# semihkacmaz/CoNFiLD

Hardware: AMD Instinct MI355X
Metric: generated fields/sec (256-step sample + CNF decode), Case4 latent, 1/2/4/8 GPU (higher is better)
Workload: dtype f32

## Files before the change

confild_amd/csrc/diffusion.hip:

```cpp
#include <cmath>
#include <string>

#include "common.hpp"
#include "sampler.hpp"

namespace cfd {

struct Philox {
    static __device__ __forceinline__ uint4 round(uint4 c, uint2 k) {
        const uint64_t p0 = (uint64_t)0xD2511F53u * c.x;
        const uint64_t p1 = (uint64_t)0xCD9E8D57u * c.z;
        return make_uint4((uint32_t)(p1 >> 32) ^ c.y ^ k.x, (uint32_t)p1, (uint32_t)(p0 >> 32) ^ c.w ^ k.y,
                          (uint32_t)p0);
    }
    static __device__ __forceinline__ uint4 gen(uint64_t seed, uint64_t ctr_lo, uint64_t ctr_hi) {
        uint4 c = make_uint4((uint32_t)ctr_lo, (uint32_t)(ctr_lo >> 32), (uint32_t)ctr_hi, (uint32_t)(ctr_hi >> 32));
        uint2 k = make_uint2((uint32_t)seed, (uint32_t)(seed >> 32));
#pragma unroll
        for (int r = 0; r < 10; ++r) {
            c = round(c, k);
            k.x += 0x9E3779B9u;
            k.y += 0xBB67AE85u;
        }
        return c;
// ... 263 lines not shown
        d_eps[i] = -g * c[CFD_COEF_SRM1];
        g_direct[i] = g * c[CFD_COEF_SRA];
    }
}

__global__ void dps_update_kernel(const float* __restrict__ sample, const float* __restrict__ g_direct,
                                  const float* __restrict__ g_unet, float scale, float* __restrict__ x_out,
                                  int64_t n) {
#pragma clang fp contract(off)
    const int64_t i = (int64_t)blockIdx.x * blockDim.x + threadIdx.x;
    if (i >= n) return;
    x_out[i] = sample[i] - (g_direct[i] + g_unet[i]) * scale;
}

struct DpsKnownArgs {
    const float* sample;
    const float* g_direct;
    const float* g_unet;
    float scale;
    float* x_out;
    const int64_t* t;
    int64_t n;
    int64_t total;
    uint64_t seed, goff;
    int vec;
};

__device__ __forceinline__ float dps_known_elem(float s, float gd, float gu, float scale, float a, float b, float kv,
                                                float m, float z2) {
#pragma clang fp contract(off)
    const float img = s - (gd + gu) * scale;
    const float q = a * kv + b * z2;
    return m * q + (1.0f - m) * img;
}

__global__ void dps_update_known_kernel(DpsKnownArgs a, KnownArgs kn) {
#pragma clang fp contract(off)
    const int64_t grp = (int64_t)blockIdx.x * blockDim.x + threadIdx.x;
    const int64_t base = grp * 4;
    if (base >= a.total) return;
    float z2[4];
    if (kn.noise2) {
        if (a.vec) {
            const f4 v = *(const f4*)(kn.noise2 + base);
            z2[0] = v.x, z2[1] = v.y, z2[2] = v.z, z2[3] = v.w;
        } else {
#pragma unroll
            for (int j = 0; j < 4; ++j) z2[j] = (base + j < a.total) ? kn.noise2[base + j] : 0.f;
        }
    } else {
        Philox::normal4(a.seed, kn.counter2, a.goff + (uint64_t)grp, z2);
    }
    if (a.vec) {
        const int64_t b = base / a.n;
        const int64_t e = base - b * a.n;
        CFD_DASSERT(base + 3 < a.total && e + 3 < a.n);
        const int64_t t = a.t[b];
        const float ta = kn.tab[t * 2], tb = kn.tab[t * 2 + 1];
        const f4 s = *(const f4*)(a.sample + base);
        const f4 gd = *(const f4*)(a.g_direct + base);
        const f4 gu = *(const f4*)(a.g_unet + base);
        const f4 kv = *(const f4*)(kn.known + b * kn.known_bstride + e);
        const f4 m = *(const f4*)(kn.mask + b * kn.mask_bstride + e);
        f4 o;
        o.x = dps_known_elem(s.x, gd.x, gu.x, a.scale, ta, tb, kv.x, m.x, z2[0]);
        o.y = dps_known_elem(s.y, gd.y, gu.y, a.scale, ta, tb, kv.y, m.y, z2[1]);
        o.z = dps_known_elem(s.z, gd.z, gu.z, a.scale, ta, tb, kv.z, m.z, z2[2]);
        o.w = dps_known_elem(s.w, gd.w, gu.w, a.scale, ta, tb, kv.w, m.w, z2[3]);
        *(f4*)(a.x_out + base) = o;
        return;
    }
#pragma unroll
    for (int j = 0; j < 4; ++j) {
        const int64_t i = base + j;
        if (i >= a.total) break;
        const int64_t b = i / a.n;
        const int64_t e = i - b * a.n;
        const int64_t t = a.t[b];
        a.x_out[i] = dps_known_elem(a.sample[i], a.g_direct[i], a.g_unet[i], a.scale, kn.tab[t * 2], kn.tab[t * 2 + 1],
                                    kn.known[b * kn.known_bstride + e], kn.mask[b * kn.mask_bstride + e], z2[j]);
    }
}

__global__ void sampler_advance_kernel(SamplerCtl* ctl, const int64_t* __restrict__ tidx_seq,
                                       const int64_t* __restrict__ tmodel_seq, int64_t* __restrict__ t_idx,
                                       int64_t* __restrict__ t_model, int B) {
    const uint64_t k = ctl->k;
    for (int b = threadIdx.x; b < B; b += blockDim.x) {
        t_idx[b] = tidx_seq[k];
        t_model[b] = tmodel_seq[k];
    }
    __syncthreads();
    if (threadIdx.x == 0) {
        ctl->counter = k;
        ctl->counter2 = CFD_KNOWN_COUNTER + k;
        ctl->counter3 = CFD_JUMP_COUNTER + k;
        ctl->k = k + 1;
    }
}

__global__ void sampler_set_kernel(SamplerCtl* ctl, uint64_t k, uint64_t seed, uint64_t goff) {
    if (threadIdx.x == 0) {
        ctl->k = k;
        ctl->counter = k;
        ctl->counter2 = CFD_KNOWN_COUNTER + k;
        ctl->counter3 = CFD_JUMP_COUNTER + k;
        ctl->seed = seed;
        ctl->goff = goff;
    }
}

}

struct cfd_sched {
    float* coefs = nullptr;
    int n_t = 0;
    int device = 0;
};

namespace cfd {
const float* sched_coefs(const cfd_sched* s) { return s->coefs; }
int sched_nt(const cfd_sched* s) { return s->n_t; }

void launch_sampler_advance(SamplerCtl* ctl, const int64_t* tidx_seq, const int64_t* tmodel_seq, int64_t* t_idx,
                            int64_t* t_model, int B, hipStream_t st) {
    hipLaunchKernelGGL(sampler_advance_kernel, dim3(1), dim3(64), 0, st, ctl, tidx_seq, tmodel_seq, t_idx, t_model, B);
    check_launch("sampler_advance_kernel");
}

void launch_sampler_set(SamplerCtl* ctl, uint64_t k, uint64_t seed, uint64_t goff, hipStream_t st) {
    hipLaunchKernelGGL(sampler_set_kernel, dim3(1), dim3(64), 0, st, ctl, k, seed, goff);
    check_launch("sampler_set_kernel");
}

void launch_sched_step_ctl(const cfd_sched* s, int kind, int clip, float* x, const float* eps, const int64_t* t,
                           const SamplerCtl* ctl, int64_t n_per_sample, int B, hipStream_t st) {
    StepArgs a{s->coefs, x, eps, t, nullptr, x, nullptr, n_per_sample, n_per_sample * B, 0, 0, 0, kind, clip, ctl};
    const int64_t groups = ceil_div(a.total, 4);
    hipLaunchKernelGGL((step_kernel<false, false>), dim3((unsigned)ceil_div(groups, 256)), dim3(256), 0, st, a, KnownArgs{},
                       JumpArgs{});
    check_launch("step_kernel");
}

void launch_sched_step_known_ctl(const cfd_sched* s, int kind, int clip, float* x, const float* eps, const int64_t* t,
                                 const SamplerCtl* ctl, const float* known, const float* mask, const float* table,
                                 int64_t n_per_sample, int B, hipStream_t st) {
    StepArgs a{s->coefs, x, eps, t, nullptr, x, nullptr, n_per_sample, n_per_sample * B, 0, 0, 0, kind, clip, ctl};
    KnownArgs kn{known, mask, n_per_sample, n_per_sample, table, nullptr, 0};
    const int64_t groups = ceil_div(a.total, 4);
    hipLaunchKernelGGL((step_kernel<true, false>), dim3((unsigned)ceil_div(groups, 256)), dim3(256), 0, st, a, kn,
                       JumpArgs{});
    check_launch("step_kernel<known>");
}

void launch_sched_step_jump_ctl(const cfd_sched* s, int kind, int clip, float* x, const float* eps, const int64_t* t,
                                const SamplerCtl* ctl, const float* known, const float* mask, const float* table,
                                const float* jtab, int n_steps, int64_t n_per_sample, int B, hipStream_t st) {
    StepArgs a{s->coefs, x, eps, t, nullptr, x, nullptr, n_per_sample, n_per_sample * B, 0, 0, 0, kind, clip, ctl};
    KnownArgs kn{known, mask, n_per_sample, n_per_sample, table, nullptr, 0};
    JumpArgs jp{1.0f, 0.0f, nullptr, 0, jtab, n_steps};
    const int64_t groups = ceil_div(a.total, 4);
    hipLaunchKernelGGL((step_kernel<true, true>), dim3((unsigned)ceil_div(groups, 256)), dim3(256), 0, st, a, kn, jp);
    check_launch("step_kernel<known, jump>");
}
}

extern "C" int cfd_sched_create(const float* host_coefs, int n_t, int device, cfd_sched** out) {
    return cfd::guard([&] {
        CFD_REQUIRE(host_coefs && out && n_t > 0, CFD_EARG, "bad argument");
        cfd::DeviceGuard dg(device);
        auto* s = new cfd_sched();
        s->n_t = n_t;
        s->device = device;
        CFD_HIP(hipMalloc(&s->coefs, sizeof(float) * n_t * CFD_NCOEF));
        CFD_HIP(hipMemcpy(s->coefs, host_coefs, sizeof(float) * n_t * CFD_NCOEF, hipMemcpyHostToDevice));
        *out = s;
    });
}

extern "C" void cfd_sched_destroy(cfd_sched* s) {
    if (!s) return;
    (void)hipFree(s->coefs);
    delete s;
}

extern "C" int cfd_sched_step(const cfd_sched* s, int kind, int clip, const float* x, const float* eps,
                              const int64_t* t, const float* noise, uint64_t seed, uint64_t counter, uint64_t offset,
                              float* x_out, float* xstart_out, int64_t n_per_sample, int B, void* stream) {
    return cfd::guard([&] {
        CFD_REQUIRE(s && x && eps && t && x_out, CFD_EARG, "null argument");
        CFD_REQUIRE(offset % 4 == 0, CFD_EARG, "noise offset must be a multiple of 4");
        CFD_REQUIRE(kind == CFD_STEP_DDPM || kind == CFD_STEP_DDIM, CFD_EARG, "unknown step kind");
        CFD_REQUIRE(n_per_sample > 0 && B > 0, CFD_EARG, "empty step");
        cfd::StepArgs a{s->coefs, x, eps, t, noise, x_out, xstart_out, n_per_sample, n_per_sample * B,
                        seed, counter, offset / 4, kind, clip, nullptr};
        const int64_t groups = cfd::ceil_div(a.total, 4);
        hipLaunchKernelGGL((cfd::step_kernel<false, false>), dim3((unsigned)cfd::ceil_div(groups, 256)), dim3(256), 0,
                           (hipStream_t)stream, a, cfd::KnownArgs{}, cfd::JumpArgs{});
        cfd::check_launch("step_kernel");
    });
}

extern "C" int cfd_sched_step_known(const cfd_sched* s, int kind, int clip, const float* x, const float* eps,
                                    const int64_t* t, const float* noise, uint64_t seed, uint64_t counter,
                                    uint64_t offset, float* x_out, float* xstart_out, int64_t n_per_sample, int B,
                                    const float* known, int64_t known_bstride, const float* mask,
                                    int64_t mask_bstride, const float* table, const float* noise2, uint64_t counter2,
                                    void* stream) {
    return cfd::guard([&] {
// ... 194 lines not shown
```

confild_amd/csrc/sampler.hip:

```cpp
#include <vector>

#include "sampler.hpp"

#include <hip/hip_ext.h>

struct cfd_sampler {
    const cfd_unet* unet = nullptr;
    const cfd_sched* sched = nullptr;
    int kind = 0, clip = 1, B = 0, n_steps = 0, device = 0, unroll = 1, graph = 1;
    int64_t n_per_sample = 0;
    float* x = nullptr;
    float* eps = nullptr;
    int64_t* tseq = nullptr;
    int64_t* tbuf = nullptr;
    cfd::SamplerCtl* ctl = nullptr;
    void* ws = nullptr;
    size_t ws_bytes = 0;
    hipGraphExec_t exec[2] = {nullptr, nullptr};
    uint64_t exec_version = ~uint64_t(0);
    float* known = nullptr;
    float* kmask = nullptr;
    float* ktab = nullptr;
    int has_known = 0;
    hipGraphExec_t kexec[2] = {nullptr, nullptr};
    float* jtab = nullptr;
    int has_jumps = 0;
    hipGraphExec_t jexec[2] = {nullptr, nullptr};
    uint64_t captures = 0;
};

namespace {

void destroy_graphs(cfd_sampler* sp) {
    for (auto* set : {sp->exec, sp->kexec, sp->jexec})
        for (int i = 0; i < 2; ++i)
            if (set[i]) {
                (void)hipGraphExecDestroy(set[i]);
                set[i] = nullptr;
            }
    sp->exec_version = ~uint64_t(0);
}

enum StepMode { STEP_PLAIN = 0, STEP_KNOWN = 1, STEP_JUMP = 2 };

void enqueue_step(const cfd_sampler* sp, StepMode mode, hipStream_t st) {
    cfd::launch_sampler_advance(sp->ctl, sp->tseq, sp->tseq + sp->n_steps, sp->tbuf, sp->tbuf + sp->B, sp->B, st);
    cfd::unet_forward_raw(sp->unet, sp->x, sp->tbuf + sp->B, sp->eps, sp->B, sp->ws, st);
    if (mode == STEP_JUMP)
        cfd::launch_sched_step_jump_ctl(sp->sched, sp->kind, sp->clip, sp->x, sp->eps, sp->tbuf, sp->ctl, sp->known,
                                        sp->kmask, sp->ktab, sp->jtab, sp->n_steps, sp->n_per_sample, sp->B, st);
    else if (mode == STEP_KNOWN)
        cfd::launch_sched_step_known_ctl(sp->sched, sp->kind, sp->clip, sp->x, sp->eps, sp->tbuf, sp->ctl, sp->known,
                                         sp->kmask, sp->ktab, sp->n_per_sample, sp->B, st);
    else
        cfd::launch_sched_step_ctl(sp->sched, sp->kind, sp->clip, sp->x, sp->eps, sp->tbuf, sp->ctl,
                                   sp->n_per_sample, sp->B, st);
}

hipGraphExec_t capture(cfd_sampler* sp, StepMode mode, int steps) {
    ++sp->captures;
    hipStream_t cs;
    CFD_HIP(hipStreamCreateWithFlags(&cs, hipStreamNonBlocking));
    hipGraph_t g = nullptr;
    hipGraphExec_t e = nullptr;
    try {
        CFD_HIP(hipStreamBeginCapture(cs, hipStreamCaptureModeThreadLocal));
        try {
            for (int i = 0; i < steps; ++i) enqueue_step(sp, mode, cs);
        } catch (...) {
            hipGraph_t dummy = nullptr;
            (void)hipStreamEndCapture(cs, &dummy);
            if (dummy) (void)hipGraphDestroy(dummy);
            throw;
        }
        CFD_HIP(hipStreamEndCapture(cs, &g));
        CFD_HIP(hipGraphInstantiate(&e, g, nullptr, nullptr, 0));
    } catch (...) {
        if (g) (void)hipGraphDestroy(g);
        (void)hipStreamDestroy(cs);
        throw;
    }
    (void)hipGraphDestroy(g);
    (void)hipStreamDestroy(cs);
    return e;
}

}

extern "C" int cfd_sampler_create(const cfd_unet* unet, const cfd_sched* sched, int kind, int clip, int B,
                                  int64_t n_per_sample, int n_steps, const int64_t* host_tidx,
                                  const int64_t* host_tmodel, int graph, int unroll, cfd_sampler** out) {
    return cfd::guard([&] {
        CFD_REQUIRE(unet && sched && out && host_tidx && host_tmodel, CFD_EARG, "null argument");
        CFD_REQUIRE(kind == CFD_STEP_DDPM || kind == CFD_STEP_DDIM, CFD_EARG, "unknown step kind");
        CFD_REQUIRE(B > 0 && n_steps > 0 && n_per_sample > 0, CFD_EARG, "empty loop");
        CFD_REQUIRE(unroll >= 1 && unroll <= 64, CFD_EARG, "unroll must be 1..64");
        cfd::unet_check_ready(unet);
        for (int k = 0; k < n_steps; ++k)
            CFD_REQUIRE(host_tidx[k] >= 0 && host_tidx[k] < cfd::sched_nt(sched), CFD_EARG,
                        "timestep index outside the coefficient table");
        cfd::DeviceGuard dg(cfd::unet_device(unet));
        auto* sp = new cfd_sampler();
        sp->unet = unet;
        sp->sched = sched;
        sp->kind = kind;
        sp->clip = clip ? 1 : 0;
        sp->B = B;
        sp->n_steps = n_steps;
        sp->n_per_sample = n_per_sample;
        sp->device = cfd::unet_device(unet);
        sp->graph = graph ? 1 : 0;
        sp->unroll = unroll;
        try {
            CFD_HIP(hipMalloc(&sp->x, sizeof(float) * (size_t)B * n_per_sample));
            CFD_HIP(hipMalloc(&sp->eps, sizeof(float) * (size_t)B * n_per_sample));
            CFD_HIP(hipMalloc(&sp->tseq, sizeof(int64_t) * 2 * (size_t)n_steps));
            CFD_HIP(hipMalloc(&sp->tbuf, sizeof(int64_t) * 2 * (size_t)B));
            CFD_HIP(hipMalloc(&sp->ctl, sizeof(cfd::SamplerCtl)));
            sp->ws_bytes = cfd::unet_ws_bytes(unet, B);
            CFD_HIP(hipMalloc(&sp->ws, sp->ws_bytes));
            CFD_HIP(hipMemcpy(sp->tseq, host_tidx, sizeof(int64_t) * n_steps, hipMemcpyHostToDevice));
            CFD_HIP(hipMemcpy(sp->tseq + n_steps, host_tmodel, sizeof(int64_t) * n_steps, hipMemcpyHostToDevice));
        } catch (...) {
            cfd_sampler_destroy(sp);
            throw;
        }
        *out = sp;
    });
}

extern "C" void cfd_sampler_destroy(cfd_sampler* sp) {
    if (!sp) return;
    destroy_graphs(sp);
    (void)hipFree(sp->x);
    (void)hipFree(sp->eps);
    (void)hipFree(sp->tseq);
    (void)hipFree(sp->tbuf);
    (void)hipFree(sp->ctl);
    (void)hipFree(sp->ws);
    (void)hipFree(sp->known);
    (void)hipFree(sp->kmask);
    (void)hipFree(sp->ktab);
    (void)hipFree(sp->jtab);
    delete sp;
}

extern "C" int cfd_sampler_run(cfd_sampler* sp, const float* x_in, float* x_out, int k0, int k1, uint64_t seed,
                               uint64_t offset, void* stream) {
    return cfd::guard([&] {
        CFD_REQUIRE(sp, CFD_EARG, "null sampler");
        CFD_REQUIRE(0 <= k0 && k0 <= k1 && k1 <= sp->n_steps, CFD_EARG, "step range outside the loop");
        CFD_REQUIRE(offset % 4 == 0, CFD_EARG, "noise offset must be a multiple of 4");
        CFD_REQUIRE(!sp->has_jumps || sp->has_known, CFD_EARG,
                    "resampling jumps need known rows (cfd_sampler_set_known)");
        cfd::unet_check_ready(sp->unet);
        cfd::DeviceGuard dg(sp->device);
        const hipStream_t st = (hipStream_t)stream;
        if (const size_t need = cfd::unet_ws_bytes(sp->unet, sp->B); need > sp->ws_bytes) {
            CFD_HIP(hipDeviceSynchronize());
            destroy_graphs(sp);
            CFD_HIP(hipFree(sp->ws));
            sp->ws = nullptr;
            sp->ws_bytes = 0;
            CFD_HIP(hipMalloc(&sp->ws, need));
            sp->ws_bytes = need;
        }
        const size_t bytes = sizeof(float) * (size_t)sp->B * sp->n_per_sample;
        if (x_in) CFD_HIP(hipMemcpyAsync(sp->x, x_in, bytes, hipMemcpyDeviceToDevice, st));
        cfd::launch_sampler_set(sp->ctl, (uint64_t)k0, seed, offset / 4, st);
        int k = k0;
        const StepMode mode = sp->has_jumps ? STEP_JUMP : sp->has_known ? STEP_KNOWN : STEP_PLAIN;
        if (sp->graph) {
            if (sp->exec_version != cfd::unet_version(sp->unet)) {
                destroy_graphs(sp);
                sp->exec_version = cfd::unet_version(sp->unet);
            }
            hipGraphExec_t* ex = mode == STEP_JUMP ? sp->jexec : mode == STEP_KNOWN ? sp->kexec : sp->exec;
            if (!ex[0]) {
                ex[0] = capture(sp, mode, 1);
                if (sp->unroll > 1) ex[1] = capture(sp, mode, sp->unroll);
            }
            for (; sp->unroll > 1 && k + sp->unroll <= k1; k += sp->unroll) CFD_HIP(hipGraphLaunch(ex[1], st));
            for (; k < k1; ++k) CFD_HIP(hipGraphLaunch(ex[0], st));
        } else {
            for (; k < k1; ++k) enqueue_step(sp, mode, st);
        }
        if (x_out) CFD_HIP(hipMemcpyAsync(x_out, sp->x, bytes, hipMemcpyDeviceToDevice, st));
    });
}

extern "C" int cfd_sampler_set_known(cfd_sampler* sp, const float* known, int64_t known_bstride, const float* mask,
                                     int64_t mask_bstride, const float* table, void* stream) {
    return cfd::guard([&] {
        CFD_REQUIRE(sp, CFD_EARG, "null sampler");
        if (!known) {
            sp->has_known = 0;
            return;
        }
        CFD_REQUIRE(mask && table, CFD_EARG, "known rows need a mask and the (n_t, 2) table");
        const int64_t n = sp->n_per_sample;
        CFD_REQUIRE((known_bstride == 0 || known_bstride == n) && (mask_bstride == 0 || mask_bstride == n), CFD_EARG,
                    "known rows and mask must be shared (stride 0) or per sample (stride n)");
        cfd::DeviceGuard dg(sp->device);
        const hipStream_t st = (hipStream_t)stream;
        const size_t row = sizeof(float) * (size_t)n, tab = sizeof(float) * 2 * (size_t)cfd::sched_nt(sp->sched);
        if (!sp->known) CFD_HIP(hipMalloc(&sp->known, row * sp->B));
        if (!sp->kmask) CFD_HIP(hipMalloc(&sp->kmask, row * sp->B));
        if (!sp->ktab) CFD_HIP(hipMalloc(&sp->ktab, tab));
        for (int b = 0; b < sp->B; ++b) {
            CFD_HIP(hipMemcpyAsync(sp->known + (size_t)b * n, known + (size_t)b * known_bstride, row,
                                   hipMemcpyDeviceToDevice, st));
            CFD_HIP(hipMemcpyAsync(sp->kmask + (size_t)b * n, mask + (size_t)b * mask_bstride, row,
                                   hipMemcpyDeviceToDevice, st));
        }
        CFD_HIP(hipMemcpyAsync(sp->ktab, table, tab, hipMemcpyDeviceToDevice, st));
        sp->has_known = 1;
    });
}

extern "C" int cfd_sampler_set_jumps(cfd_sampler* sp, const float* host_jtab) {
    return cfd::guard([&] {
        CFD_REQUIRE(sp, CFD_EARG, "null sampler");
        if (!host_jtab) {
            sp->has_jumps = 0;
            return;
        }
        for (int k = 0; k < sp->n_steps; ++k) {
            const float ja = host_jtab[2 * k], jb = host_jtab[2 * k + 1];
            CFD_REQUIRE(ja >= 0.0f && ja <= 1.0f && jb >= 0.0f && jb <= 1.0f, CFD_EARG,
                        "jump coefficients outside [0, 1]");
        }
        CFD_REQUIRE(host_jtab[2 * (sp->n_steps - 1) + 1] == 0.0f, CFD_EARG, "the last step cannot jump");
        cfd::DeviceGuard dg(sp->device);
        const size_t bytes = sizeof(float) * 2 * (size_t)sp->n_steps;
        if (!sp->jtab) CFD_HIP(hipMalloc(&sp->jtab, bytes));
        CFD_HIP(hipDeviceSynchronize());
        CFD_HIP(hipMemcpy(sp->jtab, host_jtab, bytes, hipMemcpyHostToDevice));
        sp->has_jumps = 1;
    });
}

extern "C" int cfd_sampler_captures(const cfd_sampler* sp, uint64_t* n) {
    return cfd::guard([&] {
        CFD_REQUIRE(sp && n, CFD_EARG, "null argument");
        *n = sp->captures;
    });
}

extern "C" int cfd_device_cu_count(int device, int* n_cu) {
    return cfd::guard([&] {
        CFD_REQUIRE(n_cu, CFD_EARG, "null argument");
        hipDeviceProp_t p;
// ... 26 lines not shown
```

confild_amd/csrc/sampler.hpp:

```cpp
#pragma once
#include "common.hpp"

struct cfd_unet;
struct cfd_sched;

namespace cfd {

struct SamplerCtl {
    uint64_t k;
    uint64_t counter;
    uint64_t seed;
    uint64_t goff;
    uint64_t counter2;
    uint64_t counter3;
};

constexpr uint64_t CFD_KNOWN_COUNTER = uint64_t(1) << 41;
constexpr uint64_t CFD_JUMP_COUNTER = uint64_t(1) << 42;

size_t unet_ws_bytes(const cfd_unet* h, int B);
void unet_check_ready(const cfd_unet* h);
int unet_compute(const cfd_unet* h);
uint64_t unet_version(const cfd_unet* h);
int unet_device(const cfd_unet* h);
int* unet_nonfinite(const cfd_unet* h);
void unet_forward_raw(const cfd_unet* h, const float* x, const int64_t* t, float* eps, int B, void* ws,
                      hipStream_t st);

const float* sched_coefs(const cfd_sched* s);
int sched_nt(const cfd_sched* s);
void launch_sampler_advance(SamplerCtl* ctl, const int64_t* tidx_seq, const int64_t* tmodel_seq, int64_t* t_idx,
                            int64_t* t_model, int B, hipStream_t st);
void launch_sampler_set(SamplerCtl* ctl, uint64_t k, uint64_t seed, uint64_t goff, hipStream_t st);
void launch_sched_step_ctl(const cfd_sched* s, int kind, int clip, float* x, const float* eps, const int64_t* t,
                           const SamplerCtl* ctl, int64_t n_per_sample, int B, hipStream_t st);
void launch_sched_step_known_ctl(const cfd_sched* s, int kind, int clip, float* x, const float* eps, const int64_t* t,
                                 const SamplerCtl* ctl, const float* known, const float* mask, const float* table,
                                 int64_t n_per_sample, int B, hipStream_t st);
void launch_sched_step_jump_ctl(const cfd_sched* s, int kind, int clip, float* x, const float* eps, const int64_t* t,
                                const SamplerCtl* ctl, const float* known, const float* mask, const float* table,
                                const float* jtab, int n_steps, int64_t n_per_sample, int B, hipStream_t st);

}
```

confild_amd/csrc/unet.hip:

```cpp
#include <algorithm>
#include <cstring>
#include <cmath>
#include <functional>
#include <map>
#include <string>
#include <vector>

#include "sampler.hpp"
#include "unet_kernels.hpp"
#include "unet_train.hpp"

namespace cfd {

enum class Pack { Raw, Conv3, Conv1, EmbW, EmbB };

struct UParam {
    std::string key;
    std::vector<int64_t> shape;
    Pack pack = Pack::Raw;
    size_t offset = 0;
    size_t count = 0;
    int emb_row = 0;
    bool set = false;
    int tpack = 0;
// ... 267 lines not shown
        off += nfloats * sizeof(float);
        return p;
    }
};

struct Rec {
    Act in;
    const float* h1 = nullptr;
    float *ss1 = nullptr, *st1 = nullptr;
    float *ss2 = nullptr, *st2 = nullptr;
    float *qkv = nullptr, *o = nullptr, *lse = nullptr;
    const float *act1 = nullptr, *act2 = nullptr;
    unsigned *amx1 = nullptr, *amx2 = nullptr;
    int skip_hs = -1;
    int push_hs = -1;
};

struct Tape {
    Workspace* tws;
    std::vector<Rec>* recs;
    bool keep_gnout = false;
    float* temb = nullptr;
    float* th1 = nullptr;
    float* emb = nullptr;
};

struct Sizes {
    size_t max_act = 0, max_qkv = 0, max_cat = 0, max_att = 0;
    size_t max_kvf = 0;
    size_t max_abw = 0;
    size_t max_apart = 0;
    std::vector<size_t> hs;
};

int plan_batch(const cfd_unet* h);

Sizes sizes(const cfd_unet* h) {
    const auto& c = h->cfg;
    const int mc = c.model_channels, S = c.image_size;
    Sizes z;
    int ch = c.channel_mult[0] * mc, hw = S, cmax = 0;
    z.max_act = (size_t)hw * hw * ch;
    z.hs.push_back((size_t)hw * hw * ch);
    for (int l = 0; l < c.n_mult; ++l) cmax = std::max(cmax, c.channel_mult[l] * mc);
    for (int l = 0; l < c.n_mult; ++l) {
        const int co = c.channel_mult[l] * mc;
        z.max_act = std::max(z.max_act, (size_t)hw * hw * std::max(co, ch));
        z.max_qkv = std::max(z.max_qkv, (size_t)hw * hw * 3 * co);
        z.max_cat = std::max(z.max_cat, (size_t)hw * hw * (co + cmax));
        z.max_att = std::max(z.max_att, (size_t)hw * hw * co);
        z.max_kvf = std::max(z.max_kvf, cfd::attention_split_floats(hw * hw, co));
        if (has_attn(h, 1 << l) || l == c.n_mult - 1) {
            z.max_abw = std::max(z.max_abw, cfd::attention_bwd_split_floats(hw * hw, co));
            const int heads = c.num_head_channels == -1 ? c.num_heads : co / c.num_head_channels;
            z.max_apart = std::max(z.max_apart, cfd::attention_part_floats(hw * hw, co, co / heads, plan_batch(h)));
        }
        for (int r = 0; r < c.num_res_blocks; ++r) z.hs.push_back((size_t)hw * hw * co);
        ch = co;
        if (l != c.n_mult - 1) {
            hw /= 2;
            z.hs.push_back((size_t)hw * hw * ch);
        }
    }
    z.max_cat = std::max(z.max_cat, z.max_act);
    return z;
}

constexpr size_t kSplitPer8 = size_t(16) << 20;
int plan_batch(const cfd_unet* h) { return h->plan_b > 0 ? h->plan_b : 8; }
size_t split_cap(const cfd_unet* h, int B) {
    const int pb = plan_batch(h);
    return kSplitPer8 * (size_t)std::max(1, (B + pb - 1) / pb);
}

cfd::ConvPlan plan_checked(const cfd_unet* h, const cfd::ConvArgs& a0, size_t slab_floats) {
    cfd::ConvArgs a = a0;
    a.plan_b = plan_batch(h);
    const cfd::ConvPlan p = cfd::plan_conv(a, kSplitPer8);
    CFD_REQUIRE(p.splits == 1 || (size_t)p.splits * a.M * a.Cout <= slab_floats, CFD_ESTATE,
                "internal: split-K slab too small");
    return p;
}

void run(const cfd_unet* h, const float* x, const int64_t* t, float* eps, int B, Workspace& ws, hipStream_t st,
         Tape* tape = nullptr, bool launch_req = true) {
    const auto& c = h->cfg;
    const int mc = c.model_channels, S = c.image_size;
    const Sizes z = sizes(h);
    const bool launch = launch_req && !ws.dry && !(tape && tape->tws->dry);
    const size_t kSplitCap = split_cap(h, B);
    float* temb = tape ? tape->tws->take((size_t)B * mc) : ws.take((size_t)B * mc);
    float* h1 = tape ? tape->tws->take((size_t)B * h->tdim) : ws.take((size_t)B * h->tdim);
    float* emb = tape ? tape->tws->take((size_t)B * h->tdim) : ws.take((size_t)B * h->tdim);
    if (tape) {
        tape->temb = temb;
        tape->th1 = h1;
        tape->emb = emb;
    }
    float* embo = ws.take((size_t)B * h->emb_total);
    double* gnpart = (double*)ws.take((size_t)B * cfd::kGnMaxChunks * 32 * 2 * 2);
    float* gnss = ws.take((size_t)B * 1024 * 2);
    float* nbuf = ws.take((size_t)B * z.max_cat);
    float* splitk = ws.take(kSplitCap);
    float* kvws = ws.take((size_t)B * z.max_kvf);
    float* apart = z.max_apart ? ws.take((size_t)B * z.max_apart) : nullptr;
    float* pool[3];
    for (auto& p : pool) p = ws.take((size_t)B * z.max_act);
    float* tmp = ws.take((size_t)B * z.max_act);
    float* skipb = ws.take((size_t)B * z.max_act);
    float* qkv = tape ? nullptr : ws.take((size_t)B * z.max_qkv);
    float* abuf = tape ? nullptr : ws.take((size_t)B * z.max_act);
    std::vector<float*> hsbuf;
    for (size_t n : z.hs) hsbuf.push_back(tape ? tape->tws->take((size_t)B * n) : ws.take((size_t)B * n));
    constexpr int kGnSlots = 256;
    unsigned* gslots = tape ? (unsigned*)tape->tws->take(kGnSlots) : nullptr;
    int ngs = 0;
    if (ws.dry && !tape) return;
    auto keep = [&](size_t nfloats) -> float* { return tape->tws->take(nfloats); };
    if (tape && tape->keep_gnout && launch) CFD_HIP(hipMemsetAsync(gslots, 0, sizeof(unsigned) * kGnSlots, st));
    std::vector<Rec>* recs = tape ? tape->recs : nullptr;
    if (recs) recs->assign(h->steps.size(), Rec{});

    auto pick = [&](const float* busy1, const float* busy2) -> float* {
        if (!launch && (ws.dry || !busy1)) return pool[0];
        for (auto p : pool)
            if (p != busy1 && p != busy2) return p;
        throw cfd::Error{CFD_ESTATE, "internal: buffer pool exhausted"};
    };

    if (launch) {
        cfd::launch_temb(t, h->freqs, temb, mc, B, st);
        cfd::launch_linear(temb, P(h, "time_embed.0.weight"), P(h, "time_embed.0.bias"), h1, B, mc, h->tdim, 0, st);
        cfd::launch_linear(h1, P(h, "time_embed.2.weight"), P(h, "time_embed.2.bias"), emb, B, h->tdim, h->tdim, 1,
                           st);
        cfd::launch_linear(emb, h->emb_w, h->emb_b, embo, B, h->tdim, h->emb_total, 1, st);
    }

    struct Pending {
        cfd::ConvArgs a{};
        int splits = 0;
    } pend;
    auto flush = [&]() {
        if (pend.splits > 1 && launch) cfd::launch_splitk_reduce(pend.a, pend.splits, st);
        pend.splits = 0;
    };

    auto gn = [&](const Act& in, const std::string& pre, int silu, float** ss, float** stats,
                  bool keep_raw = true, bool bf16_out = false, const float** actp = nullptr,
                  unsigned** amxp = nullptr) -> Act {
        cfd::GnArgs g{};
        g.src1 = in.a;
        g.src2 = in.b;
        g.gamma = P(h, pre + ".weight");
        g.beta = P(h, pre + ".bias");
        g.part = gnpart;
        g.ss = gnss;
        if (tape) {
            *ss = g.ss = keep((size_t)B * in.C() * 2);
            *stats = g.stats = keep((size_t)B * 64);
        }
        g.out = nbuf;
        if (tape && actp && tape->keep_gnout) {
            CFD_REQUIRE(!bf16_out && ngs < kGnSlots, CFD_ESTATE, "internal: kept GroupNorm output");
            g.out = keep((size_t)B * in.H * in.W * in.C());
            g.amax_out = gslots + ngs++;
            *actp = g.out;
            *amxp = g.amax_out;
        }
        g.C1 = in.Ca;
        g.C2 = in.Cb;
        g.Ctot = in.C();
        g.HW = in.H * in.W;
        g.eps = 1e-5f;
        g.plan_b = plan_batch(h);
        g.silu = silu;
        if (pend.splits > 1 && pend.a.out == in.a && pend.a.Cout == in.Ca && cfd::gn_takes_splitk(g, B)) {
            g.kpart = pend.a.part;
            g.ksplits = pend.splits;
            g.kbias = pend.a.bias;
            g.kemb = pend.a.emb;
            g.kemb_stride = pend.a.emb_stride;
            g.kres = pend.a.res;
            g.kx = keep_raw || cfd::gn2_applies(g) ? pend.a.out : nullptr;
            pend.splits = 0;
        } else {
            flush();
        }
        static const int gn_log = getenv("CFD_CONV_LOG") ? atoi(getenv("CFD_CONV_LOG")) : 0;
        if (gn_log && launch)
            fprintf(stderr, "GN %s %dx%d C=%d+%d ksplits=%d kres=%d kx=%d silu=%d\n", pre.c_str(), in.H, in.W, g.C1,
                    g.C2, g.kpart ? g.ksplits : 0, g.kres ? 1 : 0, g.kx ? 1 : 0, silu);
        g.out_bf16 = bf16_out ? 1 : 0;
        if (launch) cfd::launch_gn(g, B, st);
        Act r{g.out, in.C(), nullptr, 0, in.H, in.W};
        r.bf16 = bf16_out;
        return r;
    };
    auto conv_args = [&](const Act& in, const std::string& pre, int cout, int ks, int stride, int up,
                         const float* embp, const float* resp, float* out) {
        cfd::ConvArgs a{};
        a.src1 = in.a;
        a.src2 = in.b;
        a.C1 = in.Ca;
        a.C2 = in.Cb;
        a.Ctot = in.C();
        a.w = P(h, pre + ".weight");
        a.wbf = PB(h, pre + ".weight");
        a.wlo = PL(h, pre + ".weight", &a.acc_scale);
        a.bias = P(h, pre + ".bias");
        a.emb = embp;
        a.emb_stride = h->emb_total;
        a.res = resp;
        a.out = out;
        a.part = splitk;
        a.Hin = in.H;
        a.Win = in.W;
        a.Hout = up ? in.H * 2 : (stride == 2 ? (in.H + 1) / 2 : in.H);
        a.Wout = up ? in.W * 2 : (stride == 2 ? (in.W + 1) / 2 : in.W);
        a.stride = stride;
        a.ks = ks;
        a.pad = ks == 3 ? 1 : 0;
        a.up = up;
        a.Cout = cout;
        a.M = B * a.Hout * a.Wout;
        a.K = ks * ks * a.Ctot;
        a.src_bf16 = in.bf16 ? 1 : 0;
        return a;
    };
    static const int gn_bf16out = getenv("CFD_GN_BF16OUT") ? atoi(getenv("CFD_GN_BF16OUT")) : 1;
    auto feeds_k1hb = [&](const Act& in, const std::string& pre, int cout) -> bool {
        if (!gn_bf16out || h->compute != CFD_COMPUTE_BF16) return false;
        Act n{nbuf, in.C(), nullptr, 0, in.H, in.W};
        const cfd::ConvArgs a = conv_args(n, pre, cout, 3, 1, 0, nullptr, nullptr, nullptr);
        return a.wbf && !a.wlo && cfd::conv_runs_k1hb(a, plan_checked(h, a, kSplitCap));
    };
    using Tweak = std::function<void(cfd::ConvArgs&, const cfd::ConvPlan&)>;
    auto conv = [&](const Act& in, const std::string& pre, int cout, int ks, int stride, int up,
                    const float* embp, const float* resp, float* out, const Tweak& tweak = {}) {
        cfd::ConvArgs a = conv_args(in, pre, cout, ks, stride, up, embp, resp, out);
        flush();
        const cfd::ConvPlan plan = plan_checked(h, a, kSplitCap);
        if (tweak) tweak(a, plan);
        CFD_REQUIRE(!a.src_bf16 || cfd::conv_runs_k1hb(a, plan), CFD_ESTATE,
                    "internal: bf16 GroupNorm output feeds a convolution other than K1hb at " + pre);
        static const int conv_log = getenv("CFD_CONV_LOG") ? atoi(getenv("CFD_CONV_LOG")) : 0;
        if (conv_log && launch)
            fprintf(stderr, "CONV %s %dx%d C=%d+%d->%d ks=%d s=%d up=%d M=%d kx=%d bm=%d bn=%d nw=%d splits=%d\n",
                    pre.c_str(), a.Hin, a.Win, a.C1, a.C2, a.Cout, a.ks, a.stride, a.up, a.M, plan.kx, plan.bm,
                    plan.bn, plan.nw, plan.splits);
        if (launch) {
            const int sp = cfd::launch_conv(a, plan, st, true);
            if (sp > 1) {
                pend.a = a;
                pend.splits = sp;
            }
        }
    };

    std::vector<std::pair<Act, int>> stack;
    Act cur;
    size_t hs_i = 0;
    int pending_skip = -1;
    for (size_t si = 0; si < h->steps.size(); ++si) {
        const auto& s = h->steps[si];
        Rec rec;
        rec.in = cur;
        const bool to_skip = si + 1 < h->steps.size() && h->steps[si + 1].kind == cfd::Step::Push;
        auto dest = [&](const float* busy1, const float* busy2, size_t nfl) -> float* {
            if (to_skip) return hsbuf[hs_i];
            return tape ? keep(nfl) : pick(busy1, busy2);
        };
        switch (s.kind) {
            case cfd::Step::In: {
                cfd::ConvArgs a{};
                a.src1 = x;
                a.C1 = c.in_channels;
                a.Ctot = c.in_channels;
                a.w = P(h, s.conv + ".weight");
                a.bias = P(h, s.conv + ".bias");
                a.out = hsbuf[0];
                a.Hin = a.Hout = S;
                a.Win = a.Wout = S;
                a.Cout = s.cout;
                a.M = B * S * S;
                if (launch) cfd::launch_conv_in(a, st);
                cur = Act{hsbuf[0], s.cout, nullptr, 0, S, S};
                break;
            }
            case cfd::Step::Push: {
                float* dst = hsbuf[hs_i];
                if (cur.a != dst) {
                    flush();
                    if (launch)
                        CFD_HIP(hipMemcpyAsync(dst, cur.a, sizeof(float) * (size_t)B * cur.H * cur.W * cur.Ca,
// ... 886 lines not shown
                if (conv && d.tpack) {
                    CFD_REQUIRE(d.taps <= 9 && (int64_t)d.co * d.ci * d.taps == d.count, CFD_ESTATE,
                                "internal: input-gradient pack shape");
                    tiles += cfd::ceil_div(d.co, 64) * cfd::ceil_div(d.ci, cfd::RP_TI);
                }
            }
            tfirst[np] = tiles;
            CFD_HIP(hipMalloc(&h->rp_tfirst, sizeof(int64_t) * (np + 1)));
            CFD_HIP(hipMemcpy(h->rp_tfirst, tfirst.data(), sizeof(int64_t) * (np + 1), hipMemcpyHostToDevice));
            h->rp_tiles = tiles;
            CFD_HIP(hipMalloc(&h->rp_desc, sizeof(cfd::RepackDesc) * np));
            CFD_HIP(hipMalloc(&h->rp_first, sizeof(int64_t) * (np + 1)));
            CFD_HIP(hipMalloc(&h->rp_part, sizeof(float) * 2 * blocks));
            CFD_HIP(hipMalloc(&h->rp_amax, sizeof(float) * 2 * np));
            CFD_HIP(hipMemcpy(h->rp_desc, desc.data(), sizeof(cfd::RepackDesc) * np, hipMemcpyHostToDevice));
            CFD_HIP(hipMemcpy(h->rp_first, first.data(), sizeof(int64_t) * (np + 1), hipMemcpyHostToDevice));
            h->rp_blocks = blocks;
        }
        const auto* desc = (const cfd::RepackDesc*)h->rp_desc;
        hipLaunchKernelGGL(cfd::rp_amax_kernel, dim3((unsigned)h->rp_blocks), dim3(256), 0, st, flat, desc,
                           h->rp_first, np, h->rp_part);
        cfd::check_launch("rp_amax_kernel");
        hipLaunchKernelGGL(cfd::rp_reduce_kernel, dim3(np), dim3(256), 0, st, h->rp_part, h->rp_first, h->rp_amax);
        cfd::check_launch("rp_reduce_kernel");
        hipLaunchKernelGGL(cfd::rp_pack_kernel, dim3((unsigned)h->rp_blocks), dim3(256), 0, st, flat, desc,
                           h->rp_first, np, h->rp_amax, h->arena, h->arena_bf, (_Float16*)h->arena_hi,
                           (_Float16*)h->arena_lo, h->arena_t, (_Float16*)h->arena_thi, (_Float16*)h->arena_tlo,
                           h->emb_w, h->emb_b, h->tdim);
        cfd::check_launch("rp_pack_kernel");
        if (h->rp_tiles) {
            hipLaunchKernelGGL(cfd::rp_tpack_kernel, dim3((unsigned)h->rp_tiles), dim3(256), 0, st, flat, desc,
                               h->rp_tfirst, np, h->rp_amax, h->arena_t, (_Float16*)h->arena_thi,
                               (_Float16*)h->arena_tlo);
            cfd::check_launch("rp_tpack_kernel");
        }
        std::vector<float> amax(2 * (size_t)np);
        CFD_HIP(hipMemcpyAsync(amax.data(), h->rp_amax, sizeof(float) * 2 * np, hipMemcpyDeviceToHost, st));
        CFD_HIP(hipStreamSynchronize(st));
        for (int k = 0; k < np; ++k) {
            auto& p = h->params[k];
            if (p.pack == Pack::Conv1 || p.pack == Pack::Conv3) {
                int ex = 0;
                if (amax[2 * k] > 0.f) std::frexp(amax[2 * k], &ex);
                p.split_inv = std::ldexp(1.0f, ex);
            }
            if (p.tpack) {
                int ex = 0;
                if (amax[2 * k + 1] > 0.f) std::frexp(amax[2 * k + 1], &ex);
                p.tsplit_inv = std::ldexp(1.0f, ex);
            }
            p.set = true;
        }
        ++h->version;
    });
}

extern "C" int cfd_unet_set_compute(cfd_unet* h, int compute) {
    return cfd::guard([&] {
        CFD_REQUIRE(h, CFD_EARG, "null handle");
        CFD_REQUIRE(compute == CFD_COMPUTE_F32 || compute == CFD_COMPUTE_BF16 || compute == CFD_COMPUTE_SPLIT_F16,
                    CFD_EARG, "unknown compute mode");
        if (h->compute != compute) ++h->version;
        h->compute = compute;
    });
}

extern "C" int cfd_unet_set_plan_batch(cfd_unet* h, int nominal_batch) {
    return cfd::guard([&] {
        CFD_REQUIRE(h, CFD_EARG, "null handle");
        CFD_REQUIRE(nominal_batch >= 0 && nominal_batch <= 64, CFD_EARG, "plan batch must be 0 (default) .. 64");
        if (h->plan_b != nominal_batch) {
            ++h->version;
            h->ws_cache.clear();
        }
        h->plan_b = nominal_batch;
    });
}

extern "C" int cfd_unet_set_time_freqs(cfd_unet* h, const float* host, int n) {
    return cfd::guard([&] {
        CFD_REQUIRE(h && host && n == h->cfg.model_channels / 2, CFD_EARG, "freqs must have model_channels/2 entries");
        cfd::DeviceGuard dg(h->device);
        CFD_HIP(hipMemcpy(h->freqs, host, sizeof(float) * n, hipMemcpyHostToDevice));
    });
}

extern "C" int cfd_unet_ready(const cfd_unet* h) {
    return cfd::guard([&] {
        CFD_REQUIRE(h, CFD_EARG, "null handle");
        for (const auto& p : h->params) CFD_REQUIRE(p.set, CFD_ESTATE, "U-Net parameter not set: " + p.key);
    });
}

namespace cfd {
size_t unet_ws_bytes(const cfd_unet* h, int B) {
    auto it = h->ws_cache.find(B);
    if (it != h->ws_cache.end()) return it->second;
    Workspace ws{nullptr, 0, true};
    run(h, nullptr, nullptr, nullptr, B, ws, nullptr);
    h->ws_cache[B] = ws.off + 256;
    return ws.off + 256;
}
void unet_check_ready(const cfd_unet* h) {
    for (const auto& p : h->params) CFD_REQUIRE(p.set, CFD_ESTATE, "U-Net parameter not set: " + p.key);
}
int unet_compute(const cfd_unet* h) { return h->compute; }
uint64_t unet_version(const cfd_unet* h) { return h->version; }
int unet_device(const cfd_unet* h) { return h->device; }
int* unet_nonfinite(const cfd_unet* h) { return h->nonfinite; }
void unet_forward_raw(const cfd_unet* h, const float* x, const int64_t* t, float* eps, int B, void* workspace,
                      hipStream_t st) {
    Workspace ws{(char*)(((uintptr_t)workspace + 255) & ~uintptr_t(255)), 0, false};
    run(h, x, t, eps, B, ws, st);
}
}

extern "C" int cfd_unet_workspace_bytes(const cfd_unet* h, int B, size_t* bytes) {
    return cfd::guard([&] {
        CFD_REQUIRE(h && bytes && B > 0, CFD_EARG, "bad argument");
        *bytes = cfd::unet_ws_bytes(h, B);
    });
}

extern "C" int cfd_unet_forward(cfd_unet* h, const float* x, const int64_t* t, float* eps, int B, void* workspace,
                                size_t ws_bytes, void* stream) {
    return cfd::guard([&] {
        CFD_REQUIRE(h && x && t && eps && workspace, CFD_EARG, "null argument");
        CFD_REQUIRE(B > 0, CFD_EARG, "B must be positive");
        cfd::unet_check_ready(h);
        CFD_REQUIRE(ws_bytes >= cfd::unet_ws_bytes(h, B), CFD_EARG, "workspace too small");
        cfd::unet_forward_raw(h, x, t, eps, B, workspace, (hipStream_t)stream);
    });
}

namespace {
size_t tape_bytes_mode(const cfd_unet* h, int B, int mode) {
    Workspace ws{nullptr, 0, true}, tws{nullptr, 0, true};
    Tape tape{&tws, nullptr};
    tape.keep_gnout = mode == CFD_TAPE_PARAM_GRAD;
    run(h, nullptr, nullptr, nullptr, B, ws, nullptr, &tape, false);
    return tws.off + 256;
}
}

extern "C" int cfd_unet_tape_bytes(const cfd_unet* h, int B, size_t* bytes) {
    return cfd::guard([&] {
        CFD_REQUIRE(h && bytes && B > 0, CFD_EARG, "bad argument");
        *bytes = tape_bytes_mode(h, B, h->tape_mode);
    });
}

namespace {
constexpr size_t kMaxTapes = 64;

const cfd_unet::TapeRec& tape_rec(const cfd_unet* h, const void* tape, int B, size_t tape_bytes) {
    auto it = h->tapes.find(tape);
    CFD_REQUIRE(it != h->tapes.end(), CFD_ESTATE,
                "tape was not recorded by cfd_unet_forward_tape on this handle (or was forgotten: at most 64 live "
                "tapes per handle)");
    CFD_REQUIRE(it->second.B == B, CFD_EARG, "B differs from the batch the tape was recorded at");
    CFD_REQUIRE(it->second.plan == plan_batch(h), CFD_ESTATE,
                "the planned batch changed since the tape was recorded (cfd_unet_set_plan_batch)");
    CFD_REQUIRE(tape_bytes >= tape_bytes_mode(h, B, it->second.mode), CFD_EARG, "tape too small");
    return it->second;
}
}

extern "C" int cfd_unet_set_tape_mode(cfd_unet* h, int mode) {
    return cfd::guard([&] {
        CFD_REQUIRE(h, CFD_EARG, "null handle");
        CFD_REQUIRE(mode == CFD_TAPE_INPUT_VJP || mode == CFD_TAPE_PARAM_GRAD, CFD_EARG, "unknown tape mode");
        h->tape_mode = mode;
    });
}

extern "C" int cfd_unet_vjp_workspace_bytes(const cfd_unet* h, int B, size_t* bytes) {
    return cfd::guard([&] {
        CFD_REQUIRE(h && bytes && B > 0, CFD_EARG, "bad argument");
        Workspace ws{nullptr, 0, true};
        std::vector<Rec> none;
        run_vjp(h, nullptr, nullptr, B, none, ws, nullptr);
        *bytes = ws.off + 256;
    });
}

namespace {
char* align256(void* p) { return (char*)(((uintptr_t)p + 255) & ~uintptr_t(255)); }

void check_ready(const cfd_unet* h) {
    for (const auto& p : h->params) CFD_REQUIRE(p.set, CFD_ESTATE, "U-Net parameter not set: " + p.key);
}
}

extern "C" int cfd_unet_forward_tape(cfd_unet* h, const float* x, const int64_t* t, float* eps, int B,
                                     void* workspace, size_t ws_bytes, void* tape, size_t tape_bytes, void* stream) {
    return cfd::guard([&] {
// ... 94 lines not shown
```

Measured before the change: 3.778.

## Precompute timestep embedding table once and copy row per sampler step

At sampler creation, finds the distinct model timesteps and precomputes the full time-embedding MLP output (including the per-block embedding projection) for all of them into a device table. Each step's advance kernel then copies the needed row into a buffer that the U-Net reads with stride zero, skipping four small kernels per step (sinusoid embedding plus three linears). This adds table memory, a version check to refresh it when the weights or frequencies change, and a wider 1024-thread advance kernel.

```diff
diff --git a/confild_amd/csrc/diffusion.hip b/confild_amd/csrc/diffusion.hip
--- a/confild_amd/csrc/diffusion.hip
+++ b/confild_amd/csrc/diffusion.hip
@@ -369,13 +369,25 @@
     }
 }
 
-__global__ void sampler_advance_kernel(SamplerCtl* ctl, const int64_t* __restrict__ tidx_seq,
-                                       const int64_t* __restrict__ tmodel_seq, int64_t* __restrict__ t_idx,
-                                       int64_t* __restrict__ t_model, int B) {
+__global__ __launch_bounds__(1024) void sampler_advance_kernel(SamplerCtl* ctl, const int64_t* __restrict__ tidx_seq,
+                                                               const int64_t* __restrict__ tmodel_seq,
+                                                               int64_t* __restrict__ t_idx,
+                                                               int64_t* __restrict__ t_model, int B,
+                                                               const int* __restrict__ trow_seq,
+                                                               const float* __restrict__ emb_table,
+                                                               float* __restrict__ emb_row, int emb_total) {
     const uint64_t k = ctl->k;
     for (int b = threadIdx.x; b < B; b += blockDim.x) {
         t_idx[b] = tidx_seq[k];
         t_model[b] = tmodel_seq[k];
+    }
+    if (emb_table) {
+        const float* src = emb_table + (int64_t)trow_seq[k] * emb_total;
+        if (emb_total % 4 == 0) {
+            for (int i = threadIdx.x; i < emb_total / 4; i += blockDim.x) ((f4*)emb_row)[i] = ((const f4*)src)[i];
+        } else {
+            for (int i = threadIdx.x; i < emb_total; i += blockDim.x) emb_row[i] = src[i];
+        }
     }
     __syncthreads();
     if (threadIdx.x == 0) {
@@ -410,8 +422,10 @@
 int sched_nt(const cfd_sched* s) { return s->n_t; }
 
 void launch_sampler_advance(SamplerCtl* ctl, const int64_t* tidx_seq, const int64_t* tmodel_seq, int64_t* t_idx,
-                            int64_t* t_model, int B, hipStream_t st) {
-    hipLaunchKernelGGL(sampler_advance_kernel, dim3(1), dim3(64), 0, st, ctl, tidx_seq, tmodel_seq, t_idx, t_model, B);
+                            int64_t* t_model, int B, const int* trow_seq, const float* emb_table, float* emb_row,
+                            int emb_total, hipStream_t st) {
+    hipLaunchKernelGGL(sampler_advance_kernel, dim3(1), dim3(emb_table ? 1024 : 64), 0, st, ctl, tidx_seq, tmodel_seq,
+                       t_idx, t_model, B, trow_seq, emb_table, emb_row, emb_total);
     check_launch("sampler_advance_kernel");
 }
 
diff --git a/confild_amd/csrc/sampler.hip b/confild_amd/csrc/sampler.hip
--- a/confild_amd/csrc/sampler.hip
+++ b/confild_amd/csrc/sampler.hip
@@ -1,3 +1,4 @@
+#include <unordered_map>
 #include <vector>
 
 #include "sampler.hpp"
@@ -27,6 +28,13 @@
     int has_jumps = 0;
     hipGraphExec_t jexec[2] = {nullptr, nullptr};
     uint64_t captures = 0;
+    int n_distinct = 0, emb_total = 0;
+    int64_t* tdistinct = nullptr;
+    int* trow_seq = nullptr;
+    float* emb_table = nullptr;
+    float* emb_row = nullptr;
+    float* emb_scratch = nullptr;
+    uint64_t emb_version = ~uint64_t(0);
 };
 
 namespace {
@@ -44,8 +52,9 @@
 enum StepMode { STEP_PLAIN = 0, STEP_KNOWN = 1, STEP_JUMP = 2 };
 
 void enqueue_step(const cfd_sampler* sp, StepMode mode, hipStream_t st) {
-    cfd::launch_sampler_advance(sp->ctl, sp->tseq, sp->tseq + sp->n_steps, sp->tbuf, sp->tbuf + sp->B, sp->B, st);
-    cfd::unet_forward_raw(sp->unet, sp->x, sp->tbuf + sp->B, sp->eps, sp->B, sp->ws, st);
+    cfd::launch_sampler_advance(sp->ctl, sp->tseq, sp->tseq + sp->n_steps, sp->tbuf, sp->tbuf + sp->B, sp->B,
+                                sp->trow_seq, sp->emb_table, sp->emb_row, sp->emb_total, st);
+    cfd::unet_forward_raw(sp->unet, sp->x, sp->tbuf + sp->B, sp->eps, sp->B, sp->ws, st, sp->emb_row, 0);
     if (mode == STEP_JUMP)
         cfd::launch_sched_step_jump_ctl(sp->sched, sp->kind, sp->clip, sp->x, sp->eps, sp->tbuf, sp->ctl, sp->known,
                                         sp->kmask, sp->ktab, sp->jtab, sp->n_steps, sp->n_per_sample, sp->B, st);
@@ -55,6 +64,12 @@
     else
         cfd::launch_sched_step_ctl(sp->sched, sp->kind, sp->clip, sp->x, sp->eps, sp->tbuf, sp->ctl,
                                    sp->n_per_sample, sp->B, st);
+}
+
+void refresh_emb_table(cfd_sampler* sp, hipStream_t st) {
+    if (!sp->emb_table || sp->emb_version == cfd::unet_version(sp->unet)) return;
+    cfd::unet_embed(sp->unet, sp->tdistinct, sp->n_distinct, sp->emb_scratch, sp->emb_table, st);
+    sp->emb_version = cfd::unet_version(sp->unet);
 }
 
 hipGraphExec_t capture(cfd_sampler* sp, StepMode mode, int steps) {
@@ -121,6 +136,27 @@
             CFD_HIP(hipMalloc(&sp->ws, sp->ws_bytes));
             CFD_HIP(hipMemcpy(sp->tseq, host_tidx, sizeof(int64_t) * n_steps, hipMemcpyHostToDevice));
             CFD_HIP(hipMemcpy(sp->tseq + n_steps, host_tmodel, sizeof(int64_t) * n_steps, hipMemcpyHostToDevice));
+#ifndef CFD_NO_STEP_FUSE
+            std::vector<int64_t> distinct;
+            std::vector<int> trow((size_t)n_steps);
+            std::unordered_map<int64_t, int> row_of;
+            for (int k = 0; k < n_steps; ++k) {
+                const auto it = row_of.emplace(host_tmodel[k], (int)distinct.size());
+                if (it.second) distinct.push_back(host_tmodel[k]);
+                trow[(size_t)k] = it.first->second;
+            }
+            sp->n_distinct = (int)distinct.size();
+            sp->emb_total = cfd::unet_emb_total(unet);
+            CFD_HIP(hipMalloc(&sp->tdistinct, sizeof(int64_t) * distinct.size()));
+            CFD_HIP(hipMalloc(&sp->trow_seq, sizeof(int) * (size_t)n_steps));
+            CFD_HIP(hipMalloc(&sp->emb_row, sizeof(float) * (size_t)sp->emb_total));
+            CFD_HIP(hipMalloc(&sp->emb_scratch,
+                              sizeof(float) * cfd::unet_embed_scratch_floats(unet, sp->n_distinct)));
+            CFD_HIP(hipMalloc(&sp->emb_table, sizeof(float) * distinct.size() * (size_t)sp->emb_total));
+            CFD_HIP(hipMemcpy(sp->tdistinct, distinct.data(), sizeof(int64_t) * distinct.size(),
+                              hipMemcpyHostToDevice));
+            CFD_HIP(hipMemcpy(sp->trow_seq, trow.data(), sizeof(int) * (size_t)n_steps, hipMemcpyHostToDevice));
+#endif
         } catch (...) {
             cfd_sampler_destroy(sp);
             throw;
@@ -142,6 +178,11 @@
     (void)hipFree(sp->kmask);
     (void)hipFree(sp->ktab);
     (void)hipFree(sp->jtab);
+    (void)hipFree(sp->tdistinct);
+    (void)hipFree(sp->trow_seq);
+    (void)hipFree(sp->emb_table);
+    (void)hipFree(sp->emb_row);
+    (void)hipFree(sp->emb_scratch);
     delete sp;
 }
 
@@ -168,6 +209,7 @@
         const size_t bytes = sizeof(float) * (size_t)sp->B * sp->n_per_sample;
         if (x_in) CFD_HIP(hipMemcpyAsync(sp->x, x_in, bytes, hipMemcpyDeviceToDevice, st));
         cfd::launch_sampler_set(sp->ctl, (uint64_t)k0, seed, offset / 4, st);
+        refresh_emb_table(sp, st);
         int k = k0;
         const StepMode mode = sp->has_jumps ? STEP_JUMP : sp->has_known ? STEP_KNOWN : STEP_PLAIN;
         if (sp->graph) {
diff --git a/confild_amd/csrc/sampler.hpp b/confild_amd/csrc/sampler.hpp
--- a/confild_amd/csrc/sampler.hpp
+++ b/confild_amd/csrc/sampler.hpp
@@ -25,12 +25,16 @@
 int unet_device(const cfd_unet* h);
 int* unet_nonfinite(const cfd_unet* h);
 void unet_forward_raw(const cfd_unet* h, const float* x, const int64_t* t, float* eps, int B, void* ws,
-                      hipStream_t st);
+                      hipStream_t st, const float* embo = nullptr, int embo_stride = 0);
+int unet_emb_total(const cfd_unet* h);
+size_t unet_embed_scratch_floats(const cfd_unet* h, int n);
+void unet_embed(const cfd_unet* h, const int64_t* t, int n, float* scratch, float* embo, hipStream_t st);
 
 const float* sched_coefs(const cfd_sched* s);
 int sched_nt(const cfd_sched* s);
 void launch_sampler_advance(SamplerCtl* ctl, const int64_t* tidx_seq, const int64_t* tmodel_seq, int64_t* t_idx,
-                            int64_t* t_model, int B, hipStream_t st);
+                            int64_t* t_model, int B, const int* trow_seq, const float* emb_table, float* emb_row,
+                            int emb_total, hipStream_t st);
 void launch_sampler_set(SamplerCtl* ctl, uint64_t k, uint64_t seed, uint64_t goff, hipStream_t st);
 void launch_sched_step_ctl(const cfd_sched* s, int kind, int clip, float* x, const float* eps, const int64_t* t,
                            const SamplerCtl* ctl, int64_t n_per_sample, int B, hipStream_t st);
diff --git a/confild_amd/csrc/unet.hip b/confild_amd/csrc/unet.hip
--- a/confild_amd/csrc/unet.hip
+++ b/confild_amd/csrc/unet.hip
@@ -373,8 +373,17 @@
     return p;
 }
 
+void embed(const cfd_unet* h, const int64_t* t, int n, float* temb, float* h1, float* emb, float* embo,
+           hipStream_t st) {
+    const int mc = h->cfg.model_channels;
+    cfd::launch_temb(t, h->freqs, temb, mc, n, st);
+    cfd::launch_linear(temb, P(h, "time_embed.0.weight"), P(h, "time_embed.0.bias"), h1, n, mc, h->tdim, 0, st);
+    cfd::launch_linear(h1, P(h, "time_embed.2.weight"), P(h, "time_embed.2.bias"), emb, n, h->tdim, h->tdim, 1, st);
+    cfd::launch_linear(emb, h->emb_w, h->emb_b, embo, n, h->tdim, h->emb_total, 1, st);
+}
+
 void run(const cfd_unet* h, const float* x, const int64_t* t, float* eps, int B, Workspace& ws, hipStream_t st,
-         Tape* tape = nullptr, bool launch_req = true) {
+         Tape* tape = nullptr, bool launch_req = true, const float* emb_pre = nullptr, int emb_pre_stride = 0) {
     const auto& c = h->cfg;
     const int mc = c.model_channels, S = c.image_size;
     const Sizes z = sizes(h);
@@ -388,7 +397,13 @@
         tape->th1 = h1;
         tape->emb = emb;
     }
-    float* embo = ws.take((size_t)B * h->emb_total);
+    const float* embo = ws.take((size_t)B * h->emb_total);
+    int embo_stride = h->emb_total;
+    if (emb_pre) {
+        CFD_REQUIRE(!tape, CFD_ESTATE, "internal: a tape forward computes its own embeddings");
+        embo = emb_pre;
+        embo_stride = emb_pre_stride;
+    }
     double* gnpart = (double*)ws.take((size_t)B * cfd::kGnMaxChunks * 32 * 2 * 2);
     float* gnss = ws.take((size_t)B * 1024 * 2);
     float* nbuf = ws.take((size_t)B * z.max_cat);
@@ -419,13 +434,7 @@
         throw cfd::Error{CFD_ESTATE, "internal: buffer pool exhausted"};
     };
 
-    if (launch) {
-        cfd::launch_temb(t, h->freqs, temb, mc, B, st);
-        cfd::launch_linear(temb, P(h, "time_embed.0.weight"), P(h, "time_embed.0.bias"), h1, B, mc, h->tdim, 0, st);
-        cfd::launch_linear(h1, P(h, "time_embed.2.weight"), P(h, "time_embed.2.bias"), emb, B, h->tdim, h->tdim, 1,
-                           st);
-        cfd::launch_linear(emb, h->emb_w, h->emb_b, embo, B, h->tdim, h->emb_total, 1, st);
-    }
+    if (launch && !emb_pre) embed(h, t, B, temb, h1, emb, (float*)embo, st);
 
     struct Pending {
         cfd::ConvArgs a{};
@@ -500,7 +509,7 @@
         a.wlo = PL(h, pre + ".weight", &a.acc_scale);
         a.bias = P(h, pre + ".bias");
         a.emb = embp;
-        a.emb_stride = h->emb_total;
+        a.emb_stride = embo_stride;
         a.res = resp;
         a.out = out;
         a.part = splitk;
@@ -1553,6 +1562,7 @@
         CFD_REQUIRE(h && host && n == h->cfg.model_channels / 2, CFD_EARG, "freqs must have model_channels/2 entries");
         cfd::DeviceGuard dg(h->device);
         CFD_HIP(hipMemcpy(h->freqs, host, sizeof(float) * n, hipMemcpyHostToDevice));
+        ++h->version;
     });
 }
 
@@ -1580,9 +1590,18 @@
 int unet_device(const cfd_unet* h) { return h->device; }
 int* unet_nonfinite(const cfd_unet* h) { return h->nonfinite; }
 void unet_forward_raw(const cfd_unet* h, const float* x, const int64_t* t, float* eps, int B, void* workspace,
-                      hipStream_t st) {
+                      hipStream_t st, const float* embo, int embo_stride) {
     Workspace ws{(char*)(((uintptr_t)workspace + 255) & ~uintptr_t(255)), 0, false};
-    run(h, x, t, eps, B, ws, st);
+    run(h, x, t, eps, B, ws, st, nullptr, true, embo, embo_stride);
+}
+int unet_emb_total(const cfd_unet* h) { return h->emb_total; }
+size_t unet_embed_scratch_floats(const cfd_unet* h, int n) {
+    return (size_t)n * (h->cfg.model_channels + 2 * (size_t)h->tdim);
+}
+void unet_embed(const cfd_unet* h, const int64_t* t, int n, float* scratch, float* embo, hipStream_t st) {
+    float* temb = scratch;
+    float* h1 = temb + (size_t)n * h->cfg.model_channels;
+    embed(h, t, n, temb, h1, h1 + (size_t)n * h->tdim, embo, st);
 }
 }
 
```

Measured after the change: 3.786, median of 6. No clear change (+0.2%).
